# AhauBioinformatics/IDDGCN

Measured on AMD Instinct MI355X. Metric: adjacency edges/s per IDDGCN training step (pos fwd + neg fwd + bwd + Adam), higher is better.
Workload: dtype f32

## Files before the change

### iddgcn_amd/csrc/iddgcn_hip.hip

```cpp
#include <hip/hip_runtime.h>
#include <stdint.h>

#include <type_traits>

#include "../../include/iddgcn.h"

typedef float f32x4 __attribute__((ext_vector_type(4)));
typedef float f32x16 __attribute__((ext_vector_type(16)));
typedef _Float16 f16x4 __attribute__((ext_vector_type(4)));
typedef _Float16 f16x8 __attribute__((ext_vector_type(8)));
typedef __bf16 bf16x8 __attribute__((ext_vector_type(8)));
typedef __bf16 bf16x4 __attribute__((ext_vector_type(4)));
typedef short s16x4 __attribute__((ext_vector_type(4)));
typedef unsigned int u32x2 __attribute__((ext_vector_type(2)));
typedef unsigned int u32x4 __attribute__((ext_vector_type(4)));

#define MAX_R 8
#define EPS_BCE 1e-7f

namespace {

__device__ __forceinline__ float sigmoidf_(float x) { return 1.0f / (1.0f + expf(-x)); }
__device__ __forceinline__ float sigmoid_fast(float x) { return __builtin_amdgcn_rcpf(1.0f + __expf(-x)); }

// ... 2191 lines not shown
            tr_read_asm(fa[k][1], pa + 512 * k + 4 * PT);
            tr_read_asm(fb[k][0], pb0 + 512 * k);
            tr_read_asm(fb[k][1], pb0 + 512 * k + 4 * PT);
        }
        tie6(fa);
        tie6(fb);
        const bf16x8 a0 = frag(fa[0]), a1 = frag(fa[1]), a2 = frag(fa[2]);
#pragma unroll
        for (int cj = 0; cj < 8; ++cj) {
            if (cj + 1 < 8) {
                const char* pb = pb0 + 64 * (cj + 1);
#pragma unroll
                for (int k = 0; k < 3; ++k) {
                    tr_read_asm(fn[k][0], pb + 512 * k);
                    tr_read_asm(fn[k][1], pb + 512 * k + 4 * PT);
                }
            }
            const bf16x8 b0 = frag(fb[0]), b1 = frag(fb[1]), b2 = frag(fb[2]);
            f32x16 c;
#pragma unroll
            for (int j = 0; j < 16; ++j) c[j] = 0.f;
            c = __builtin_amdgcn_mfma_f32_32x32x16_bf16(a0, b2, c, 0, 0, 0);
            c = __builtin_amdgcn_mfma_f32_32x32x16_bf16(a2, b0, c, 0, 0, 0);
            c = __builtin_amdgcn_mfma_f32_32x32x16_bf16(a1, b1, c, 0, 0, 0);
            c = __builtin_amdgcn_mfma_f32_32x32x16_bf16(a0, b1, c, 0, 0, 0);
            c = __builtin_amdgcn_mfma_f32_32x32x16_bf16(a1, b0, c, 0, 0, 0);
            acc[cj] = __builtin_amdgcn_mfma_f32_32x32x16_bf16(a0, b0, acc[cj] + c, 0, 0, 0);
            __builtin_amdgcn_sched_barrier(0);
            if (cj + 1 < 8) {
                tie6(fn);
#pragma unroll
                for (int k = 0; k < 3; ++k) {
                    fb[k][0] = fn[k][0];
                    fb[k][1] = fn[k][1];
                }
            }
        }
    };

    if (nt > 0) {
        stage(0, 0);
        const int n1 = nt > 1 ? stage(1, 1) : 0;
        wait_newest(n1);
        convert(0);
        asm volatile("s_waitcnt lgkmcnt(0)" ::: "memory");
        __syncthreads();
    }
#define TB3_LOOP(LATE)                                                               \
    {                                                                                \
        int b = 0;                                                                   \
        for (long long t = 0; t < nt; ++t) {                                         \
            const int b1 = b == 2 ? 0 : b + 1, b2 = b1 == 2 ? 0 : b1 + 1;            \
            const int n2 = t + 2 < nt ? stage(t + 2, b2) : 0;                        \
            if (LATE && t + 1 < nt) {                                                \
                wait_newest(n2);                                                     \
                convert(b1);                                                         \
            }                                                                        \
            mfma_tile(b);                                                            \
            if (!LATE && t + 1 < nt) {                                               \
                wait_newest(n2);                                                     \
                convert(b1);                                                         \
            }                                                                        \
            asm volatile("s_waitcnt lgkmcnt(0)" ::: "memory");                       \
            __builtin_amdgcn_s_barrier();                                            \
            asm volatile("" ::: "memory");                                           \
            b = b1;                                                                  \
        }                                                                            \
    }
    if (late) TB3_LOOP(true) else TB3_LOOP(false)
#undef TB3_LOOP
    float* out = slab + (long long)blockIdx.x * D * D;
    const int i = lane & 31, h = lane >> 5;
#pragma unroll
    for (int cj = 0; cj < 8; ++cj)
#pragma unroll
        for (int j = 0; j < 16; ++j) {
            const int row = 32 * wave + (j & 3) + 8 * (j >> 2) + 4 * h;
            out[row * D + 32 * cj + i] = acc[cj][j];
        }
}

namespace st3 {
constexpr int D = 256, TR = 32, DP = 1536, XP = 768, DOB = TR * DP, XB = TR * XP, BUF = DOB + XB, NBUF = 2;
}
template <int PS>
__device__ __forceinline__ void tr_read3(v4s16 (&d)[3], unsigned a) {
    asm volatile("ds_read_b64_tr_b16 %0, %3\n\tds_read_b64_tr_b16 %1, %3 offset:%4\n\tds_read_b64_tr_b16 %2, %3 offset:%5"
                 : "=&v"(d[0]), "=&v"(d[1]), "=&v"(d[2])
                 : "v"(a), "i"(PS), "i"(2 * PS)
                 : "memory");
}
__device__ __forceinline__ bf16x8 cat_tr(const v4s16& a, const v4s16& b) {
    return __builtin_bit_cast(bf16x8, __builtin_shufflevector(a, b, 0, 1, 2, 3, 4, 5, 6, 7));
}
__device__ __forceinline__ float bf_at(const u32x2& v, int q) {
    const unsigned w = v[q >> 1];
    return __builtin_bit_cast(float, (q & 1) ? (w & 0xffff0000u) : (w << 16));
}
__global__ __launch_bounds__(512) void sigma_tn_b3_kernel(long long M, int tiles_per_block, int n_ranges,
                                                          const float* __restrict__ dO, float* __restrict__ X,
                                                          const float* __restrict__ S, float* __restrict__ slab) {
    using namespace st3;
    static_assert(NBUF * BUF <= 160 * 1024, "LDS budget");
    __shared__ __attribute__((aligned(16))) char lds[NBUF * BUF];
    const int lane = threadIdx.x & 63;
    const int wave = __builtin_amdgcn_readfirstlane(threadIdx.x >> 6);
    const int bx = blockIdx.x;
    const int half = (bx >> 3) & 1;
    const int range = ((bx >> 4) << 3) | (bx & 7);
    if (range >= n_ranges) return;
    const long long ntiles = (M + TR - 1) / TR;
    const long long t_beg = (long long)range * tiles_per_block;
    long long t_end = t_beg + tiles_per_block;
    if (t_end > ntiles) t_end = ntiles;
    const int i16 = lane & 15, g = lane >> 4;
    const int c0 = 128 * half + 16 * wave;
    const unsigned lds0 = lds_u32(lds);
    auto fresh_lane = [&]() __attribute__((always_inline)) {
        int l = lane;
        asm volatile("" : "+v"(l));
        return l;
    };

    bf16x8 w0[8], w1[8], w2[8];
#pragma unroll
    for (int q = 0; q < 8; ++q)
#pragma unroll
        for (int e = 0; e < 8; ++e) {
            __bf16 a, b, c;
            split3(S[(c0 + i16) * D + 32 * q + 8 * g + e], a, b, c);
            w0[q][e] = a;
            w1[q][e] = b;
            w2[q][e] = c;
        }
    f32x4 tacc[2][8];
#pragma unroll
    for (int mb = 0; mb < 2; ++mb)
#pragma unroll
        for (int nb = 0; nb < 8; ++nb) tacc[mb][nb] = f32x4{0.f, 0.f, 0.f, 0.f};

    auto stage = [&](long long t, int bb, int wave) __attribute__((always_inline)) -> int {
        const int lane = fresh_lane();
        char* base = lds + bb * BUF;
        const long long t0 = t * TR;
        if (t0 + TR <= M) {
#pragma unroll
            for (int j = 0; j < 4; ++j) {
                const int r = 4 * wave + j;
                __builtin_amdgcn_global_load_lds((gbl_vptr)(dO + (t0 + r) * D + lane * 4), (lds_vptr)(base + r * DP), 16,
                                                 0, 0);
            }
#pragma unroll
            for (int p = 0; p < 2; ++p) {
                const int r = 4 * wave + 2 * p;
                __builtin_amdgcn_global_load_lds(
                    (gbl_vptr)(X + (t0 + r + (lane >> 5)) * D + 128 * half + (lane & 31) * 4),
                    (lds_vptr)(base + DOB + r * XP), 16, 0, 0);
            }
            return 6;
        }
        int n = 0;
#pragma unroll
        for (int j = 0; j < 4; ++j) {
            const int r = 4 * wave + j;
            const long long e = t0 + r;
            char* xr = base + DOB + (r & ~1) * XP + 512 * (r & 1);
            if (e < M) {
                __builtin_amdgcn_global_load_lds((gbl_vptr)(dO + e * D + lane * 4), (lds_vptr)(base + r * DP), 16, 0, 0);
                if (lane < 32)
                    __builtin_amdgcn_global_load_lds((gbl_vptr)(X + e * D + 128 * half + lane * 4), (lds_vptr)xr, 16, 0,
                                                     0);
                n += 2;
            } else {
                st4(reinterpret_cast<float*>(base + r * DP) + lane * 4, f32x4{0.f, 0.f, 0.f, 0.f});
                if (lane < 32) st4(reinterpret_cast<float*>(xr) + lane * 4, f32x4{0.f, 0.f, 0.f, 0.f});
            }
        }
        return n;
    };
    auto convert = [&](int bb, int wave) __attribute__((always_inline)) {
        char* base = lds + bb * BUF;
        const int lane = fresh_lane();
        u32x4 v[6];
#pragma unroll
        for (int j = 0; j < 4; ++j)
            asm volatile("ds_read_b128 %0, %1" : "=v"(v[j]) : "v"(lds_u32(base + (4 * wave + j) * DP) + 16 * lane) : "memory");
#pragma unroll
        for (int p = 0; p < 2; ++p)
            asm volatile("ds_read_b128 %0, %1"
                         : "=v"(v[4 + p])
                         : "v"(lds_u32(base + DOB + (4 * wave + 2 * p) * XP) + 16 * lane)
                         : "memory");
        asm volatile("s_waitcnt lgkmcnt(0)" : "+v"(v[0]), "+v"(v[1]), "+v"(v[2]), "+v"(v[3]), "+v"(v[4]), "+v"(v[5])::"memory");
#pragma unroll
        for (int j = 0; j < 4; ++j) {
            const int r = 4 * wave + j;
            char* row = base + r * DP + 16 * ((lane >> 1) ^ stn_sw(r)) + 8 * (lane & 1);
            bf16x4 p0, p1, p2;
            split3x4(__builtin_bit_cast(f32x4, v[j]), p0, p1, p2);
            *reinterpret_cast<bf16x4*>(row) = p0;
            *reinterpret_cast<bf16x4*>(row + 512) = p1;
            *reinterpret_cast<bf16x4*>(row + 1024) = p2;
        }
#pragma unroll
        for (int p = 0; p < 2; ++p) {
            const int r = 4 * wave + 2 * p + (lane >> 5);
            char* row = base + DOB + r * XP + 16 * (((lane & 31) >> 1) ^ stn_sw(r)) + 8 * (lane & 1);
            bf16x4 p0, p1, p2;
            split3x4(__builtin_bit_cast(f32x4, v[4 + p]), p0, p1, p2);
            *reinterpret_cast<bf16x4*>(row) = p0;
            *reinterpret_cast<bf16x4*>(row + 256) = p1;
            *reinterpret_cast<bf16x4*>(row + 512) = p2;
        }
    };
    auto mfma_sigma = [&](int bb, f32x4 (&acc)[2]) __attribute__((always_inline)) {
        const int lane = fresh_lane();
        const int i16 = lane & 15, g = lane >> 4, swi = stn_sw(i16), sa = swi >> 2, sl = swi & 3;
        const unsigned rb0 = lds0 + bb * BUF + i16 * DP + 16 * (g ^ sl);
        const unsigned ad0 = rb0 + 64 * (0 ^ sa), ad1 = rb0 + 64 * (1 ^ sa), ad2 = rb0 + 64 * (2 ^ sa),
                       ad3 = rb0 + 64 * (3 ^ sa);
        f32x4 hi0 = {0.f, 0.f, 0.f, 0.f}, lo0 = hi0, hi1 = hi0, lo1 = hi0;
        u32x4 fx[2][3], fy[2][3];
        asm volatile("s_waitcnt lgkmcnt(0)" ::: "memory");
#define ST3_LOADQ(Q, S_, AD)                                                                              \
        asm volatile("ds_read_b128 %0, %6 offset:%7\n\tds_read_b128 %1, %6 offset:%8\n\t"                 \
                     "ds_read_b128 %2, %6 offset:%9\n\tds_read_b128 %3, %6 offset:%10\n\t"                \
                     "ds_read_b128 %4, %6 offset:%11\n\tds_read_b128 %5, %6 offset:%12"                   \
                     : "=&v"(fx[S_][0]), "=&v"(fx[S_][1]), "=&v"(fx[S_][2]), "=&v"(fy[S_][0]), "=&v"(fy[S_][1]),  \
                       "=&v"(fy[S_][2])                                                                  \
                     : "v"(AD), "i"(256 * ((Q) >> 2)), "i"(256 * ((Q) >> 2) + 512),                       \
                       "i"(256 * ((Q) >> 2) + 1024), "i"(256 * ((Q) >> 2) + 16 * DP),                     \
                       "i"(256 * ((Q) >> 2) + 16 * DP + 512), "i"(256 * ((Q) >> 2) + 16 * DP + 1024)      \
                     : "memory")
        ST3_LOADQ(0, 0, ad0);
#pragma unroll
        for (int q = 0; q < 8; ++q) {
            const int S_ = q & 1;
            if (q + 1 < 8) {
                switch (q) {
                    case 0: ST3_LOADQ(1, 1, ad1); break;
                    case 1: ST3_LOADQ(2, 0, ad2); break;
                    case 2: ST3_LOADQ(3, 1, ad3); break;
                    case 3: ST3_LOADQ(4, 0, ad0); break;
                    case 4: ST3_LOADQ(5, 1, ad1); break;
                    case 5: ST3_LOADQ(6, 0, ad2); break;
                    default: ST3_LOADQ(7, 1, ad3); break;
                }
                asm volatile("s_waitcnt lgkmcnt(6)"
                             : "+v"(fx[S_][0]), "+v"(fx[S_][1]), "+v"(fx[S_][2]), "+v"(fy[S_][0]), "+v"(fy[S_][1]),
                               "+v"(fy[S_][2])::"memory");
            } else {
                asm volatile("s_waitcnt lgkmcnt(0)"
                             : "+v"(fx[S_][0]), "+v"(fx[S_][1]), "+v"(fx[S_][2]), "+v"(fy[S_][0]), "+v"(fy[S_][1]),
                               "+v"(fy[S_][2])::"memory");
            }
            const bf16x8 x0 = __builtin_bit_cast(bf16x8, fx[S_][0]), x1 = __builtin_bit_cast(bf16x8, fx[S_][1]),
                         x2 = __builtin_bit_cast(bf16x8, fx[S_][2]);
            const bf16x8 y0 = __builtin_bit_cast(bf16x8, fy[S_][0]), y1 = __builtin_bit_cast(bf16x8, fy[S_][1]),
                         y2 = __builtin_bit_cast(bf16x8, fy[S_][2]);
            lo0 = __builtin_amdgcn_mfma_f32_16x16x32_bf16(w0[q], x2, lo0, 0, 0, 0);
            lo1 = __builtin_amdgcn_mfma_f32_16x16x32_bf16(w0[q], y2, lo1, 0, 0, 0);
            lo0 = __builtin_amdgcn_mfma_f32_16x16x32_bf16(w2[q], x0, lo0, 0, 0, 0);
            lo1 = __builtin_amdgcn_mfma_f32_16x16x32_bf16(w2[q], y0, lo1, 0, 0, 0);
            lo0 = __builtin_amdgcn_mfma_f32_16x16x32_bf16(w1[q], x1, lo0, 0, 0, 0);
            lo1 = __builtin_amdgcn_mfma_f32_16x16x32_bf16(w1[q], y1, lo1, 0, 0, 0);
            lo0 = __builtin_amdgcn_mfma_f32_16x16x32_bf16(w0[q], x1, lo0, 0, 0, 0);
            lo1 = __builtin_amdgcn_mfma_f32_16x16x32_bf16(w0[q], y1, lo1, 0, 0, 0);
            lo0 = __builtin_amdgcn_mfma_f32_16x16x32_bf16(w1[q], x0, lo0, 0, 0, 0);
            lo1 = __builtin_amdgcn_mfma_f32_16x16x32_bf16(w1[q], y0, lo1, 0, 0, 0);
            hi0 = __builtin_amdgcn_mfma_f32_16x16x32_bf16(w0[q], x0, hi0, 0, 0, 0);
            hi1 = __builtin_amdgcn_mfma_f32_16x16x32_bf16(w0[q], y0, hi1, 0, 0, 0);
        }
#undef ST3_LOADQ
        acc[0] = hi0 + lo0;
        acc[1] = hi1 + lo1;
    };
    auto mfma_tn = [&](int bb) __attribute__((always_inline)) {
        const int lane = fresh_lane();
        const int tra = 8 * (lane >> 4) + ((lane >> 2) & 3), trq = tra + 4;
        const int swa = stn_sw(tra), swq = stn_sw(trq);
        const int tb = (lane & 3) >> 1;
        const unsigned xoa = tra * XP + 16 * (tb ^ (swa & 1)) + 8 * (lane & 1),
                       xoq = trq * XP + 16 * (tb ^ (swq & 1)) + 8 * (lane & 1);
        const unsigned doa = tra * DP + 16 * (tb ^ (swa & 1)) + 8 * (lane & 1) + 256 * (wave >> 2),
                       doq = trq * DP + 16 * (tb ^ (swq & 1)) + 8 * (lane & 1) + 256 * (wave >> 2);
        const int swa_e = swa & 14, swq_e = swq & 14;
        const unsigned db = lds0 + bb * BUF, xb = db + DOB;
        v4s16 xa[2][2][3], fb[2][2][3];
#pragma unroll
        for (int mb = 0; mb < 2; ++mb) {
            const int cx = 4 * (wave & 3) + 2 * mb;
            tr_read3<256>(xa[mb][0], xb + xoa + 16 * (cx ^ swa_e));
            tr_read3<256>(xa[mb][1], xb + xoq + 16 * (cx ^ swq_e));
        }
        tr_read3<512>(fb[0][0], db + doa + 16 * (0 ^ swa_e));
        tr_read3<512>(fb[0][1], db + doq + 16 * (0 ^ swq_e));
        asm volatile("s_waitcnt lgkmcnt(0)"
                     : "+v"(xa[0][0][0]), "+v"(xa[0][0][1]), "+v"(xa[0][0][2]), "+v"(xa[0][1][0]), "+v"(xa[0][1][1]),
                       "+v"(xa[0][1][2]), "+v"(xa[1][0][0]), "+v"(xa[1][0][1]), "+v"(xa[1][0][2]), "+v"(xa[1][1][0]),
                       "+v"(xa[1][1][1]), "+v"(xa[1][1][2]), "+v"(fb[0][0][0]), "+v"(fb[0][0][1]), "+v"(fb[0][0][2]),
                       "+v"(fb[0][1][0]), "+v"(fb[0][1][1]), "+v"(fb[0][1][2])::"memory");
        bf16x8 a[2][3];
#pragma unroll
        for (int mb = 0; mb < 2; ++mb)
#pragma unroll
            for (int j = 0; j < 3; ++j) a[mb][j] = cat_tr(xa[mb][0][j], xa[mb][1][j]);
#pragma unroll
        for (int nb = 0; nb < 8; ++nb) {
            const int s = nb & 1;
            if (nb + 1 < 8) {
                tr_read3<512>(fb[s ^ 1][0], db + doa + 16 * ((2 * (nb + 1)) ^ swa_e));
                tr_read3<512>(fb[s ^ 1][1], db + doq + 16 * ((2 * (nb + 1)) ^ swq_e));
            }
            const bf16x8 b0 = cat_tr(fb[s][0][0], fb[s][1][0]), b1 = cat_tr(fb[s][0][1], fb[s][1][1]),
                         b2 = cat_tr(fb[s][0][2], fb[s][1][2]);
            const f32x4 z = {0.f, 0.f, 0.f, 0.f};
            f32x4 e0 = __builtin_amdgcn_mfma_f32_16x16x32_bf16(a[0][0], b2, z, 0, 0, 0);
            f32x4 e1 = __builtin_amdgcn_mfma_f32_16x16x32_bf16(a[1][0], b2, z, 0, 0, 0);
            e0 = __builtin_amdgcn_mfma_f32_16x16x32_bf16(a[0][2], b0, e0, 0, 0, 0);
            e1 = __builtin_amdgcn_mfma_f32_16x16x32_bf16(a[1][2], b0, e1, 0, 0, 0);
            e0 = __builtin_amdgcn_mfma_f32_16x16x32_bf16(a[0][1], b1, e0, 0, 0, 0);
            e1 = __builtin_amdgcn_mfma_f32_16x16x32_bf16(a[1][1], b1, e1, 0, 0, 0);
            e0 = __builtin_amdgcn_mfma_f32_16x16x32_bf16(a[0][0], b1, e0, 0, 0, 0);
            e1 = __builtin_amdgcn_mfma_f32_16x16x32_bf16(a[1][0], b1, e1, 0, 0, 0);
            e0 = __builtin_amdgcn_mfma_f32_16x16x32_bf16(a[0][1], b0, e0, 0, 0, 0);
            e1 = __builtin_amdgcn_mfma_f32_16x16x32_bf16(a[1][1], b0, e1, 0, 0, 0);
            tacc[0][nb] = __builtin_amdgcn_mfma_f32_16x16x32_bf16(a[0][0], b0, tacc[0][nb] + e0, 0, 0, 0);
            tacc[1][nb] = __builtin_amdgcn_mfma_f32_16x16x32_bf16(a[1][0], b0, tacc[1][nb] + e1, 0, 0, 0);
            __builtin_amdgcn_sched_barrier(0);
            if (nb + 1 < 8)
                asm volatile("s_waitcnt lgkmcnt(0)"
                             : "+v"(fb[s ^ 1][0][0]), "+v"(fb[s ^ 1][0][1]), "+v"(fb[s ^ 1][0][2]), "+v"(fb[s ^ 1][1][0]),
                               "+v"(fb[s ^ 1][1][1]), "+v"(fb[s ^ 1][1][2])::"memory");
        }
    };
    auto epilogue = [&](long long t, int bb, const f32x4 (&acc)[2]) __attribute__((always_inline)) -> int {
        const int lane = fresh_lane();
        const int i16 = lane & 15, g = lane >> 4, swi = stn_sw(i16);
        const unsigned xb = lds0 + bb * BUF + DOB + 16 * ((2 * wave + (g >> 1)) ^ swi) + 8 * (g & 1);
        u32x2 xr[2][3];
#pragma unroll
        for (int rb = 0; rb < 2; ++rb)
            asm volatile("ds_read_b64 %0, %3\n\tds_read_b64 %1, %3 offset:256\n\tds_read_b64 %2, %3 offset:512"
                         : "=&v"(xr[rb][0]), "=&v"(xr[rb][1]), "=&v"(xr[rb][2])
                         : "v"(xb + (16 * rb + i16) * XP)
                         : "memory");
        asm volatile("s_waitcnt lgkmcnt(0)"
                     : "+v"(xr[0][0]), "+v"(xr[0][1]), "+v"(xr[0][2]), "+v"(xr[1][0]), "+v"(xr[1][1]), "+v"(xr[1][2])::"memory");
        const long long row0 = t * TR;
        const long long left = M - row0;
        const unsigned nbytes = (unsigned)((left < TR ? left : TR) * D * 4);
        const __amdgpu_buffer_rsrc_t rc =
            __builtin_amdgcn_make_buffer_rsrc(reinterpret_cast<char*>(X) + row0 * D * 4, (short)0, nbytes, 0x00020000);
#pragma unroll
        for (int rb = 0; rb < 2; ++rb) {
            const int r = 16 * rb + i16;
            f32x4 v = acc[rb];
#pragma unroll
            for (int q = 0; q < 4; ++q) {
                const float x = (bf_at(xr[rb][0], q) + bf_at(xr[rb][1], q)) + bf_at(xr[rb][2], q);
                v[q] = v[q] * (x * (1.0f - x));
            }
            __builtin_amdgcn_raw_buffer_store_b128(v, rc, (r * D + 128 * half + 16 * wave + 4 * g) * 4, 0, 0);
        }
        return 2;
    };

    if (t_beg < t_end) {
        stage(t_beg, 0, wave);
        asm volatile("s_waitcnt vmcnt(0)" ::: "memory");
        convert(0, wave);
        asm volatile("s_waitcnt lgkmcnt(0)" ::: "memory");
        __syncthreads();
        {
            int b = 0;
            const bool stager = wave < 4;
            for (long long t = t_beg; t < t_end; ++t) {
                const bool more = t + 1 < t_end;
                if (more && stager) {
                    stage(t + 1, b ^ 1, wave);
                    stage(t + 1, b ^ 1, wave + 4);
                }
                f32x4 acc[2];
                mfma_sigma(b, acc);
                const int ns = epilogue(t, b, acc);
                mfma_tn(b);
                if (more && stager) {
                    wait_vm(ns);
                    convert(b ^ 1, wave);
                    convert(b ^ 1, wave + 4);
                }
                asm volatile("s_waitcnt lgkmcnt(0)" ::: "memory");
                __builtin_amdgcn_s_barrier();
                asm volatile("" ::: "memory");
                b ^= 1;
            }
        }
    }
    float* out = slab + (long long)range * D * D;
#pragma unroll
    for (int mb = 0; mb < 2; ++mb)
#pragma unroll
        for (int nb = 0; nb < 8; ++nb)
#pragma unroll
            for (int j = 0; j < 4; ++j) {
                const int row = 128 * half + 32 * (wave & 3) + 16 * mb + 4 * g + j;
                out[row * D + 128 * (wave >> 2) + 16 * nb + i16] = tacc[mb][nb][j];
            }
}

template <int D>
__global__ __launch_bounds__(D) void gemm_tn_narrow_kernel(long long M, long long rows_per_block, int R,
                                                           const float* __restrict__ A,
                                                           const float* __restrict__ dz,
                                                           float* __restrict__ slab) {
    const int d = threadIdx.x;
    float acc[MAX_R], accb[MAX_R];
#pragma unroll
    for (int r = 0; r < MAX_R; ++r) acc[r] = accb[r] = 0.f;
    const long long r_beg = (long long)blockIdx.x * rows_per_block;
    long long r_end = r_beg + rows_per_block;
    if (r_end > M) r_end = M;
    for (long long e = r_beg; e < r_end; ++e) {
        const float a = A[e * D + d];
#pragma unroll
        for (int r = 0; r < MAX_R; ++r)
            if (r < R) {
                const float z = dz[e * R + r];
                acc[r] += a * z;
                accb[r] += z;
            }
    }
    float* out = slab + (long long)blockIdx.x * (D + 1) * R;
#pragma unroll
    for (int r = 0; r < MAX_R; ++r)
        if (r < R) {
            out[d * R + r] = acc[r];
            if (d == 0) out[D * R + r] = accb[r];
        }
}

template <int D>
__global__ __launch_bounds__(256) void alpha_kernel(int M, int R, const float* __restrict__ X,
                                                    const int* __restrict__ x_idx, const float* __restrict__ Wa,
                                                    const float* __restrict__ ba, float* __restrict__ S_out,
                                                    float* __restrict__ W_out) {
    constexpr int LPR = D / 4;
    constexpr int K = LPR < MAX_R ? LPR : MAX_R;
    const int sub = threadIdx.x % LPR;
    float wa[4][MAX_R];
#pragma unroll
    for (int j = 0; j < 4; ++j)
#pragma unroll
        for (int r = 0; r < MAX_R; ++r) wa[j][r] = r < R ? Wa[(sub * 4 + j) * R + r] : 0.f;
    float bav[MAX_R];
#pragma unroll
    for (int r = 0; r < MAX_R; ++r) bav[r] = r < R ? ba[r] : 0.f;
    const long long gstride = (long long)gridDim.x * (blockDim.x / LPR);
    for (long long row = ((long long)blockIdx.x * blockDim.x + threadIdx.x) / LPR; row < M; row += gstride) {
        const long long src = x_idx ? (long long)x_idx[row] : row;
        const f32x4 x = ld4(X + src * D + sub * 4);
        float z[MAX_R];
#pragma unroll
        for (int r0 = 0; r0 < MAX_R; r0 += K) {
            float part[K];
#pragma unroll
            for (int q = 0; q < K; ++q) {
                const int r = r0 + q;
                part[q] = 0.f;
#pragma unroll
                for (int j = 0; j < 4; ++j) part[q] = fmaf(x[j], wa[j][r], part[q]);
            }
            const float tot = multi_reduce<LPR, K>(part, sub);
#pragma unroll
            for (int q = 0; q < K; ++q) z[r0 + q] = __shfl(tot, (threadIdx.x & ~(LPR - 1) & 63) + q * (LPR / K), 64);
        }
        if (sub != 0) continue;
        float mx = -INFINITY;
#pragma unroll
        for (int r = 0; r < MAX_R; ++r)
            if (r < R) {
                z[r] += bav[r];
                mx = fmaxf(mx, z[r]);
            }
        float sum = 0.f;
#pragma unroll
        for (int r = 0; r < MAX_R; ++r)
            if (r < R) {
                z[r] = expf(z[r] - mx);
                sum += z[r];
// ... 2150 lines not shown
    if (a->planes) return IDDGCN_E_BAD_ARG;
    RowGemmP p = to_p(*a);
    p.accumulate = 0;
    auto al16 = [](const void* q) { return ((uintptr_t)q & 15) == 0; };
    if (a->R == 8 && a->v_idx && !a->coef_idx && !a->a_idx && !a->b_trans && !dsig && al16(a->A) && al16(a->C) &&
        al16(a->coef) && al16(a->V) && (a->v_rel_stride & 3) == 0) {
        launch_fwd_gather8((hipStream_t)stream, p);
        return launch_status();
    }
    V3Sel sel;
    sel.nv = a->R == 0 ? 0 : a->R == 1 ? 1 : a->R == 2 ? 2 : a->R <= 4 ? 4 : 8;
    sel.aux = dsig;
    sel.hc = a->R > 0;
    RowGemmBatch pb;
    pb.p[0] = p;
    launch_v3((hipStream_t)stream, pb, 1, sel, true);
    return launch_status();
}

int iddgcn_gemm_tn_bf16(void* stream, long long M, int d, const void* A, const void* B, float* slab, int n_blocks,
                        float* C, int accumulate) {
    if (d != 256) return IDDGCN_E_BAD_DIM;
    if (M < 0 || n_blocks < 1 || !A || !B || !slab || !C) return IDDGCN_E_BAD_ARG;
    hipStream_t st = (hipStream_t)stream;
    long long rpb = (M + n_blocks - 1) / n_blocks;
    rpb = ((rpb + 31) / 32) * 32;
    if (rpb < 32) rpb = 32;
    hipLaunchKernelGGL(gemm_tn256_bf16t_kernel, dim3(n_blocks), dim3(512), 0, st, M, rpb,
                       (const __bf16*)A, (const __bf16*)B, slab);
    int rc = launch_status();
    if (rc) return rc;
    const long long n = (long long)d * d;
    launch_reduce_slabs(st, n_blocks, n, slab, C, accumulate, 1.0f);
    return launch_status();
}

int iddgcn_sigma_tn_ranges(long long M) {
    const long long nt = (M + stn::TR - 1) / stn::TR;
    long long nr = nt < 128 ? nt : 128;
    if (nr < 1) nr = 1;
    const long long tpb = (nt + nr - 1) / nr > 0 ? (nt + nr - 1) / nr : 1;
    nr = (nt + tpb - 1) / tpb;
    return (int)((nr + 7) / 8 * 8 > 0 ? (nr + 7) / 8 * 8 : 8);
}

int iddgcn_sigma_tn_bf16(void* stream, long long M, int d, const void* dO, void* X, const float* S, float* slab,
                         long long slab_floats, float* dS, int precision) {
    if (d != 256) return IDDGCN_E_BAD_DIM;
    if (precision != IDDGCN_GEMM_EXACT_F32 && precision != IDDGCN_GEMM_SPLIT_F16 && precision != IDDGCN_GEMM_BF16X3 &&
        precision != IDDGCN_GEMM_BF16)
        return IDDGCN_E_BAD_ARG;
    if (M < 0 || !S || !slab || !dS || (M > 0 && (!dO || !X))) return IDDGCN_E_BAD_ARG;
    if (((uintptr_t)dO & 15) || ((uintptr_t)X & 15)) return IDDGCN_E_BAD_ARG;
    hipStream_t st = (hipStream_t)stream;
    const long long nt = (M + stn::TR - 1) / stn::TR;
    const int nr = iddgcn_sigma_tn_ranges(M);
    const long long tpb = nt > 0 ? (nt + nr - 1) / nr : 1;
    const long long n = (long long)d * d;
    if (slab_floats < nr * n) return IDDGCN_E_BAD_ARG;
    if (precision == IDDGCN_GEMM_BF16)
        hipLaunchKernelGGL(sigma_tn_bf16_kernel<true>, dim3((unsigned)(2 * nr)), dim3(512), 0, st, M, (int)tpb, nr,
                           (const __bf16*)dO, (__bf16*)X, S, slab);
    else
        hipLaunchKernelGGL(sigma_tn_bf16_kernel<false>, dim3((unsigned)(2 * nr)), dim3(512), 0, st, M, (int)tpb, nr,
                           (const __bf16*)dO, (__bf16*)X, S, slab);
    int rc = launch_status();
    if (rc) return rc;
    launch_reduce_slabs(st, nr, n, slab, dS, 0, 1.0f);
    return launch_status();
}

int iddgcn_sigma_tn_f32(void* stream, long long M, int d, const float* dO, float* X, const float* S, float* slab,
                        long long slab_floats, float* dS, int precision) {
    if (d != 256) return IDDGCN_E_BAD_DIM;
    if (precision != IDDGCN_GEMM_BF16X3) return IDDGCN_E_BAD_ARG;
    if (M < 0 || !S || !slab || !dS || (M > 0 && (!dO || !X))) return IDDGCN_E_BAD_ARG;
    if (((uintptr_t)dO & 15) || ((uintptr_t)X & 15)) return IDDGCN_E_BAD_ARG;
    hipStream_t st = (hipStream_t)stream;
    const long long nt = (M + st3::TR - 1) / st3::TR;
    const int nr = iddgcn_sigma_tn_ranges(M);
    const long long tpb = nt > 0 ? (nt + nr - 1) / nr : 1;
    const long long n = (long long)d * d;
    if (slab_floats < nr * n) return IDDGCN_E_BAD_ARG;
    hipLaunchKernelGGL(sigma_tn_b3_kernel, dim3((unsigned)(2 * nr)), dim3(512), 0, st, M, (int)tpb, nr, dO, X, S, slab);
    int rc = launch_status();
    if (rc) return rc;
    launch_reduce_slabs(st, nr, n, slab, dS, 0, 1.0f);
    return launch_status();
}

int iddgcn_combine_bf16(void* stream, int M, int d, int R, const float* Y, const int* idx, const float* coef,
                        const float* V, long long v_rel_stride, void* out) {
    return run_combine_out<true, false>(stream, M, d, R, Y, idx, coef, V, v_rel_stride, out);
}

int iddgcn_combine_planes_f32(void* stream, int M, int d, int R, const float* Y, const int* idx, const float* coef,
                              const float* V, long long v_rel_stride, void* out) {
    return run_combine_out<false, true>(stream, M, d, R, Y, idx, coef, V, v_rel_stride, out);
}

int iddgcn_distmult_bce_bf16(void* stream, long long T, int d, int R, const float* Xh, const int* h_idx,
                             const void* Xt, const int* t_idx, const int* r_idx, const float* rel, const float* y,
                             float scale, float* p_out, float* s_out, float* ds_out, void* do_out,
                             float* drel_slab, float* loss_slab, int n_blocks) {
    if (d != 256) return IDDGCN_E_BAD_DIM;
    if (R < 1 || R > MAX_R) return IDDGCN_E_BAD_REL;
    if (T < 0 || n_blocks < 1 || !Xh || !h_idx || !Xt || !r_idx || !rel) return IDDGCN_E_BAD_ARG;
    if (y && (!ds_out || !do_out || !drel_slab || !loss_slab)) return IDDGCN_E_BAD_ARG;
    if (T == 0) return 0;
    hipLaunchKernelGGL((distmult_kernel<256, true>), dim3(n_blocks), dim3(256), 0, (hipStream_t)stream, T, R, Xh, h_idx,
                       (const float*)Xt, t_idx, r_idx, rel, y, scale, p_out, s_out, ds_out, (float*)do_out, drel_slab,
                       loss_slab);
    return launch_status();
}

int iddgcn_distmult_bce_heads_bf16(void* stream, int n_nodes, int d, int R, const int* seg_ptr, const int* perm,
                                   const float* Xh, const void* Xt, const int* r_idx, const float* rel,
                                   const float* y, float scale, float* p_out, float* s_out, float* ds_out,
                                   void* do_out, float* dXh, float* drel_slab, float* loss_slab, int n_blocks) {
    if (d != 256) return IDDGCN_E_BAD_DIM;
    if (R < 1 || R > MAX_R) return IDDGCN_E_BAD_REL;
    if (n_nodes < 0 || n_blocks < 1 || !seg_ptr || !perm || !Xh || !Xt || !r_idx || !rel || !do_out || !dXh ||
        !drel_slab || !loss_slab)
        return IDDGCN_E_BAD_ARG;
    hipStream_t st = (hipStream_t)stream;
#define HKB(RT) hipLaunchKernelGGL((distmult_heads_kernel<256, RT, true>), dim3(n_blocks), dim3(256), 0, st, n_nodes, R, seg_ptr, perm, Xh, (const float*)Xt, r_idx, rel, y, scale, p_out, s_out, ds_out, (float*)do_out, dXh, drel_slab, loss_slab)
    if (R <= 1) HKB(1);
    else if (R <= 2) HKB(2);
    else if (R <= 4) HKB(4);
    else HKB(8);
#undef HKB
    return launch_status();
}

int iddgcn_tail_seg_reduce_head_bf16(void* stream, int n_nodes, int d, int R, const int* seg_ptr, const float* W,
                                     const void* dO, const float* P, long long p_rel_stride, float* dP,
                                     long long dp_rel_stride, float* dsum, float* dWedge, const float* head_dO,
                                     const float* Wn, float* dwh) {
    if (d != 256) return IDDGCN_E_BAD_DIM;
    if (R != 8) return IDDGCN_E_BAD_REL;
    if (n_nodes < 0 || !seg_ptr || !W || !dO || !P || !dP || !dWedge || !head_dO || !Wn || !dwh)
        return IDDGCN_E_BAD_ARG;
    if (n_nodes == 0) return 0;
    launch_tail_mfma8((hipStream_t)stream, n_nodes, seg_ptr, W, dO, P, p_rel_stride, dP, dp_rel_stride, dsum, dWedge,
                      head_dO, Wn, dwh);
    return launch_status();
}

int iddgcn_head_dz_f32(void* stream, int n_nodes, int R, const float* Ssm, const float* W, const int* hseg_ptr,
                       const int* hperm, const float* dWedge, const float* dwh, float* dz) {
    if (R < 1 || R > MAX_R) return IDDGCN_E_BAD_REL;
    if (n_nodes < 0 || !Ssm || !W || !hseg_ptr || !hperm || !dWedge || !dwh || !dz) return IDDGCN_E_BAD_ARG;
    if (n_nodes == 0) return 0;
    hipLaunchKernelGGL(head_dz_kernel, dim3((unsigned)(((long long)n_nodes * 8 + 255) / 256)), dim3(256), 0,
                       (hipStream_t)stream, n_nodes, R, Ssm, W, hseg_ptr, hperm, dWedge, dwh, dz);
    return launch_status();
}

int iddgcn_tail_seg_reduce_bf16(void* stream, int n_nodes, int d, int R, const int* seg_ptr, const int* h_idx,
                                const float* W, const void* dO, const float* P, long long p_rel_stride, float* dP,
                                long long dp_rel_stride, float* dsum, float* dWedge) {
    if (d != 256) return IDDGCN_E_BAD_DIM;
    if (R < 1 || R > MAX_R) return IDDGCN_E_BAD_REL;
    if (n_nodes < 0 || !seg_ptr || !W || !dO || !P || !dP || !dWedge) return IDDGCN_E_BAD_ARG;
    if (n_nodes == 0) return 0;
    hipStream_t st = (hipStream_t)stream;
    const unsigned grid = grid_for(n_nodes, 64);
// ... 29 lines not shown
```

Before: 81.46 million.

## Add dedicated TN waves to sigma_tn kernel and rebalance column work

Raises the fused sigma/TN backward kernel from 8 to 12 waves per block. The 4 new waves only compute the X^T·dO product for 12 of the 16 column blocks, while the original 8 waves keep the sigma MFMA, epilogue and staging and handle the remaining 4 column blocks. The goal is to take most of the TN accumulation off the critical path of the sigma waves so the two matrix products overlap. The sigma LDS reads are also reorganised into a finer-grained interleaved prefetch between MFMA groups. The cost is higher register pressure from the 768-thread launch bound and a larger block, which may reduce occupancy.

```diff
diff --git a/iddgcn_amd/csrc/iddgcn_hip.hip b/iddgcn_amd/csrc/iddgcn_hip.hip
--- a/iddgcn_amd/csrc/iddgcn_hip.hip
+++ b/iddgcn_amd/csrc/iddgcn_hip.hip
@@ -2297,6 +2297,11 @@
 
 namespace st3 {
 constexpr int D = 256, TR = 32, DP = 1536, XP = 768, DOB = TR * DP, XB = TR * XP, BUF = DOB + XB, NBUF = 2;
+constexpr int NBT = 12;
+template <int N>
+struct ic {
+    static constexpr int v = N;
+};
 }
 template <int PS>
 __device__ __forceinline__ void tr_read3(v4s16 (&d)[3], unsigned a) {
@@ -2312,7 +2317,7 @@
     const unsigned w = v[q >> 1];
     return __builtin_bit_cast(float, (q & 1) ? (w & 0xffff0000u) : (w << 16));
 }
-__global__ __launch_bounds__(512) void sigma_tn_b3_kernel(long long M, int tiles_per_block, int n_ranges,
+__global__ __launch_bounds__(768) void sigma_tn_b3_kernel(long long M, int tiles_per_block, int n_ranges,
                                                           const float* __restrict__ dO, float* __restrict__ X,
                                                           const float* __restrict__ S, float* __restrict__ slab) {
     using namespace st3;
@@ -2328,7 +2333,7 @@
     const long long t_beg = (long long)range * tiles_per_block;
     long long t_end = t_beg + tiles_per_block;
     if (t_end > ntiles) t_end = ntiles;
-    const int i16 = lane & 15, g = lane >> 4;
+    const int n_t = __builtin_amdgcn_readfirstlane(t_end > t_beg ? (int)(t_end - t_beg) : 0);
     const int c0 = 128 * half + 16 * wave;
     const unsigned lds0 = lds_u32(lds);
     auto fresh_lane = [&]() __attribute__((always_inline)) {
@@ -2337,22 +2342,8 @@
         return l;
     };
 
+    const bool tn_wave = wave >= 8;
     bf16x8 w0[8], w1[8], w2[8];
-#pragma unroll
-    for (int q = 0; q < 8; ++q)
-#pragma unroll
-        for (int e = 0; e < 8; ++e) {
-            __bf16 a, b, c;
-            split3(S[(c0 + i16) * D + 32 * q + 8 * g + e], a, b, c);
-            w0[q][e] = a;
-            w1[q][e] = b;
-            w2[q][e] = c;
-        }
-    f32x4 tacc[2][8];
-#pragma unroll
-    for (int mb = 0; mb < 2; ++mb)
-#pragma unroll
-        for (int nb = 0; nb < 8; ++nb) tacc[mb][nb] = f32x4{0.f, 0.f, 0.f, 0.f};
 
     auto stage = [&](long long t, int bb, int wave) __attribute__((always_inline)) -> int {
         const int lane = fresh_lane();
@@ -2431,85 +2422,78 @@
     auto mfma_sigma = [&](int bb, f32x4 (&acc)[2]) __attribute__((always_inline)) {
         const int lane = fresh_lane();
         const int i16 = lane & 15, g = lane >> 4, swi = stn_sw(i16), sa = swi >> 2, sl = swi & 3;
-        const unsigned rb0 = lds0 + bb * BUF + i16 * DP + 16 * (g ^ sl);
-        const unsigned ad0 = rb0 + 64 * (0 ^ sa), ad1 = rb0 + 64 * (1 ^ sa), ad2 = rb0 + 64 * (2 ^ sa),
-                       ad3 = rb0 + 64 * (3 ^ sa);
+        const unsigned sb = lds0 + bb * BUF, rb0 = i16 * DP + 16 * (g ^ sl) + 64 * sa;
+        auto adq = [&](int q) __attribute__((always_inline)) {
+            unsigned r = rb0;
+            asm volatile("" : "+v"(r));
+            return sb + 256 * (q >> 2) + (r ^ (64 * (q & 3)));
+        };
         f32x4 hi0 = {0.f, 0.f, 0.f, 0.f}, lo0 = hi0, hi1 = hi0, lo1 = hi0;
-        u32x4 fx[2][3], fy[2][3];
+        u32x4 x0, y0, x1, y1, x2, y2;
         asm volatile("s_waitcnt lgkmcnt(0)" ::: "memory");
-#define ST3_LOADQ(Q, S_, AD)                                                                              \
-        asm volatile("ds_read_b128 %0, %6 offset:%7\n\tds_read_b128 %1, %6 offset:%8\n\t"                 \
-                     "ds_read_b128 %2, %6 offset:%9\n\tds_read_b128 %3, %6 offset:%10\n\t"                \
-                     "ds_read_b128 %4, %6 offset:%11\n\tds_read_b128 %5, %6 offset:%12"                   \
-                     : "=&v"(fx[S_][0]), "=&v"(fx[S_][1]), "=&v"(fx[S_][2]), "=&v"(fy[S_][0]), "=&v"(fy[S_][1]),  \
-                       "=&v"(fy[S_][2])                                                                  \
-                     : "v"(AD), "i"(256 * ((Q) >> 2)), "i"(256 * ((Q) >> 2) + 512),                       \
-                       "i"(256 * ((Q) >> 2) + 1024), "i"(256 * ((Q) >> 2) + 16 * DP),                     \
-                       "i"(256 * ((Q) >> 2) + 16 * DP + 512), "i"(256 * ((Q) >> 2) + 16 * DP + 1024)      \
-                     : "memory")
-        ST3_LOADQ(0, 0, ad0);
+#define ST3_LD2(DX, DY, AD, OFF)                                                                               \
+        do {                                                                                                   \
+            asm volatile("ds_read_b128 %0, %1 offset:%2" : "=v"(DX) : "v"(AD), "i"(OFF) : "memory");           \
+            asm volatile("ds_read_b128 %0, %1 offset:%2" : "=v"(DY) : "v"(AD), "i"((OFF) + 16 * DP) : "memory"); \
+        } while (0)
+        {
+            const unsigned ad = adq(0);
+            ST3_LD2(x0, y0, ad, 0);
+            ST3_LD2(x2, y2, ad, 1024);
+            ST3_LD2(x1, y1, ad, 512);
+        }
 #pragma unroll
         for (int q = 0; q < 8; ++q) {
-            const int S_ = q & 1;
-            if (q + 1 < 8) {
-                switch (q) {
-                    case 0: ST3_LOADQ(1, 1, ad1); break;
-                    case 1: ST3_LOADQ(2, 0, ad2); break;
-                    case 2: ST3_LOADQ(3, 1, ad3); break;
-                    case 3: ST3_LOADQ(4, 0, ad0); break;
-                    case 4: ST3_LOADQ(5, 1, ad1); break;
-                    case 5: ST3_LOADQ(6, 0, ad2); break;
-                    default: ST3_LOADQ(7, 1, ad3); break;
-                }
-                asm volatile("s_waitcnt lgkmcnt(6)"
-                             : "+v"(fx[S_][0]), "+v"(fx[S_][1]), "+v"(fx[S_][2]), "+v"(fy[S_][0]), "+v"(fy[S_][1]),
-                               "+v"(fy[S_][2])::"memory");
-            } else {
-                asm volatile("s_waitcnt lgkmcnt(0)"
-                             : "+v"(fx[S_][0]), "+v"(fx[S_][1]), "+v"(fx[S_][2]), "+v"(fy[S_][0]), "+v"(fy[S_][1]),
-                               "+v"(fy[S_][2])::"memory");
-            }
-            const bf16x8 x0 = __builtin_bit_cast(bf16x8, fx[S_][0]), x1 = __builtin_bit_cast(bf16x8, fx[S_][1]),
-                         x2 = __builtin_bit_cast(bf16x8, fx[S_][2]);
-            const bf16x8 y0 = __builtin_bit_cast(bf16x8, fy[S_][0]), y1 = __builtin_bit_cast(bf16x8, fy[S_][1]),
-                         y2 = __builtin_bit_cast(bf16x8, fy[S_][2]);
-            lo0 = __builtin_amdgcn_mfma_f32_16x16x32_bf16(w0[q], x2, lo0, 0, 0, 0);
-            lo1 = __builtin_amdgcn_mfma_f32_16x16x32_bf16(w0[q], y2, lo1, 0, 0, 0);
-            lo0 = __builtin_amdgcn_mfma_f32_16x16x32_bf16(w2[q], x0, lo0, 0, 0, 0);
-            lo1 = __builtin_amdgcn_mfma_f32_16x16x32_bf16(w2[q], y0, lo1, 0, 0, 0);
-            lo0 = __builtin_amdgcn_mfma_f32_16x16x32_bf16(w1[q], x1, lo0, 0, 0, 0);
-            lo1 = __builtin_amdgcn_mfma_f32_16x16x32_bf16(w1[q], y1, lo1, 0, 0, 0);
-            lo0 = __builtin_amdgcn_mfma_f32_16x16x32_bf16(w0[q], x1, lo0, 0, 0, 0);
-            lo1 = __builtin_amdgcn_mfma_f32_16x16x32_bf16(w0[q], y1, lo1, 0, 0, 0);
-            lo0 = __builtin_amdgcn_mfma_f32_16x16x32_bf16(w1[q], x0, lo0, 0, 0, 0);
-            lo1 = __builtin_amdgcn_mfma_f32_16x16x32_bf16(w1[q], y0, lo1, 0, 0, 0);
-            hi0 = __builtin_amdgcn_mfma_f32_16x16x32_bf16(w0[q], x0, hi0, 0, 0, 0);
-            hi1 = __builtin_amdgcn_mfma_f32_16x16x32_bf16(w0[q], y0, hi1, 0, 0, 0);
-        }
-#undef ST3_LOADQ
+            const bool more = q + 1 < 8;
+            const unsigned nad = adq(more ? q + 1 : q);
+            asm volatile("s_waitcnt lgkmcnt(0)" : "+v"(x0), "+v"(y0), "+v"(x2), "+v"(y2), "+v"(x1), "+v"(y1)::"memory");
+            const bf16x8 fx0 = __builtin_bit_cast(bf16x8, x0), fy0 = __builtin_bit_cast(bf16x8, y0);
+            const bf16x8 fx1 = __builtin_bit_cast(bf16x8, x1), fy1 = __builtin_bit_cast(bf16x8, y1);
+            lo0 = __builtin_amdgcn_mfma_f32_16x16x32_bf16(w0[q], __builtin_bit_cast(bf16x8, x2), lo0, 0, 0, 0);
+            lo1 = __builtin_amdgcn_mfma_f32_16x16x32_bf16(w0[q], __builtin_bit_cast(bf16x8, y2), lo1, 0, 0, 0);
+            __builtin_amdgcn_sched_barrier(0);
+            if (more) ST3_LD2(x2, y2, nad, 1024);
+            lo0 = __builtin_amdgcn_mfma_f32_16x16x32_bf16(w2[q], fx0, lo0, 0, 0, 0);
+            lo1 = __builtin_amdgcn_mfma_f32_16x16x32_bf16(w2[q], fy0, lo1, 0, 0, 0);
+            lo0 = __builtin_amdgcn_mfma_f32_16x16x32_bf16(w1[q], fx1, lo0, 0, 0, 0);
+            lo1 = __builtin_amdgcn_mfma_f32_16x16x32_bf16(w1[q], fy1, lo1, 0, 0, 0);
+            lo0 = __builtin_amdgcn_mfma_f32_16x16x32_bf16(w0[q], fx1, lo0, 0, 0, 0);
+            lo1 = __builtin_amdgcn_mfma_f32_16x16x32_bf16(w0[q], fy1, lo1, 0, 0, 0);
+            __builtin_amdgcn_sched_barrier(0);
+            if (more) ST3_LD2(x1, y1, nad, 512);
+            lo0 = __builtin_amdgcn_mfma_f32_16x16x32_bf16(w1[q], fx0, lo0, 0, 0, 0);
+            lo1 = __builtin_amdgcn_mfma_f32_16x16x32_bf16(w1[q], fy0, lo1, 0, 0, 0);
+            hi0 = __builtin_amdgcn_mfma_f32_16x16x32_bf16(w0[q], fx0, hi0, 0, 0, 0);
+            hi1 = __builtin_amdgcn_mfma_f32_16x16x32_bf16(w0[q], fy0, hi1, 0, 0, 0);
+            __builtin_amdgcn_sched_barrier(0);
+            if (more) ST3_LD2(x0, y0, nad, 0);
+        }
+#undef ST3_LD2
         acc[0] = hi0 + lo0;
         acc[1] = hi1 + lo1;
     };
-    auto mfma_tn = [&](int bb) __attribute__((always_inline)) {
+    auto mfma_tn = [&](int bb, int xg, int nb0, auto nbc, auto dbc, auto& tacc) __attribute__((always_inline)) {
+        constexpr int NB = decltype(nbc)::v;
+        constexpr bool DB = decltype(dbc)::v != 0;
         const int lane = fresh_lane();
         const int tra = 8 * (lane >> 4) + ((lane >> 2) & 3), trq = tra + 4;
         const int swa = stn_sw(tra), swq = stn_sw(trq);
         const int tb = (lane & 3) >> 1;
         const unsigned xoa = tra * XP + 16 * (tb ^ (swa & 1)) + 8 * (lane & 1),
                        xoq = trq * XP + 16 * (tb ^ (swq & 1)) + 8 * (lane & 1);
-        const unsigned doa = tra * DP + 16 * (tb ^ (swa & 1)) + 8 * (lane & 1) + 256 * (wave >> 2),
-                       doq = trq * DP + 16 * (tb ^ (swq & 1)) + 8 * (lane & 1) + 256 * (wave >> 2);
+        const unsigned doa = tra * DP + 16 * (tb ^ (swa & 1)) + 8 * (lane & 1),
+                       doq = trq * DP + 16 * (tb ^ (swq & 1)) + 8 * (lane & 1);
         const int swa_e = swa & 14, swq_e = swq & 14;
         const unsigned db = lds0 + bb * BUF, xb = db + DOB;
         v4s16 xa[2][2][3], fb[2][2][3];
 #pragma unroll
         for (int mb = 0; mb < 2; ++mb) {
-            const int cx = 4 * (wave & 3) + 2 * mb;
+            const int cx = 4 * xg + 2 * mb;
             tr_read3<256>(xa[mb][0], xb + xoa + 16 * (cx ^ swa_e));
             tr_read3<256>(xa[mb][1], xb + xoq + 16 * (cx ^ swq_e));
         }
-        tr_read3<512>(fb[0][0], db + doa + 16 * (0 ^ swa_e));
-        tr_read3<512>(fb[0][1], db + doq + 16 * (0 ^ swq_e));
+        tr_read3<512>(fb[0][0], db + doa + 16 * ((2 * nb0) ^ swa_e));
+        tr_read3<512>(fb[0][1], db + doq + 16 * ((2 * nb0) ^ swq_e));
         asm volatile("s_waitcnt lgkmcnt(0)"
                      : "+v"(xa[0][0][0]), "+v"(xa[0][0][1]), "+v"(xa[0][0][2]), "+v"(xa[0][1][0]), "+v"(xa[0][1][1]),
                        "+v"(xa[0][1][2]), "+v"(xa[1][0][0]), "+v"(xa[1][0][1]), "+v"(xa[1][0][2]), "+v"(xa[1][1][0]),
@@ -2521,11 +2505,12 @@
 #pragma unroll
             for (int j = 0; j < 3; ++j) a[mb][j] = cat_tr(xa[mb][0][j], xa[mb][1][j]);
 #pragma unroll
-        for (int nb = 0; nb < 8; ++nb) {
-            const int s = nb & 1;
-            if (nb + 1 < 8) {
-                tr_read3<512>(fb[s ^ 1][0], db + doa + 16 * ((2 * (nb + 1)) ^ swa_e));
-                tr_read3<512>(fb[s ^ 1][1], db + doq + 16 * ((2 * (nb + 1)) ^ swq_e));
+        for (int i = 0; i < NB; ++i) {
+            const int s = DB ? (i & 1) : 0, sn = DB ? (s ^ 1) : 0;
+            const bool more = i + 1 < NB;
+            if (DB && more) {
+                tr_read3<512>(fb[sn][0], db + doa + 16 * ((2 * (nb0 + i + 1)) ^ swa_e));
+                tr_read3<512>(fb[sn][1], db + doq + 16 * ((2 * (nb0 + i + 1)) ^ swq_e));
             }
             const bf16x8 b0 = cat_tr(fb[s][0][0], fb[s][1][0]), b1 = cat_tr(fb[s][0][1], fb[s][1][1]),
                          b2 = cat_tr(fb[s][0][2], fb[s][1][2]);
@@ -2540,13 +2525,17 @@
             e1 = __builtin_amdgcn_mfma_f32_16x16x32_bf16(a[1][0], b1, e1, 0, 0, 0);
             e0 = __builtin_amdgcn_mfma_f32_16x16x32_bf16(a[0][1], b0, e0, 0, 0, 0);
             e1 = __builtin_amdgcn_mfma_f32_16x16x32_bf16(a[1][1], b0, e1, 0, 0, 0);
-            tacc[0][nb] = __builtin_amdgcn_mfma_f32_16x16x32_bf16(a[0][0], b0, tacc[0][nb] + e0, 0, 0, 0);
-            tacc[1][nb] = __builtin_amdgcn_mfma_f32_16x16x32_bf16(a[1][0], b0, tacc[1][nb] + e1, 0, 0, 0);
+            tacc[0][i] = __builtin_amdgcn_mfma_f32_16x16x32_bf16(a[0][0], b0, tacc[0][i] + e0, 0, 0, 0);
+            tacc[1][i] = __builtin_amdgcn_mfma_f32_16x16x32_bf16(a[1][0], b0, tacc[1][i] + e1, 0, 0, 0);
             __builtin_amdgcn_sched_barrier(0);
-            if (nb + 1 < 8)
+            if (!DB && more) {
+                tr_read3<512>(fb[0][0], db + doa + 16 * ((2 * (nb0 + i + 1)) ^ swa_e));
+                tr_read3<512>(fb[0][1], db + doq + 16 * ((2 * (nb0 + i + 1)) ^ swq_e));
+            }
+            if (more)
                 asm volatile("s_waitcnt lgkmcnt(0)"
-                             : "+v"(fb[s ^ 1][0][0]), "+v"(fb[s ^ 1][0][1]), "+v"(fb[s ^ 1][0][2]), "+v"(fb[s ^ 1][1][0]),
-                               "+v"(fb[s ^ 1][1][1]), "+v"(fb[s ^ 1][1][2])::"memory");
+                             : "+v"(fb[sn][0][0]), "+v"(fb[sn][0][1]), "+v"(fb[sn][0][2]), "+v"(fb[sn][1][0]),
+                               "+v"(fb[sn][1][1]), "+v"(fb[sn][1][2])::"memory");
         }
     };
     auto epilogue = [&](long long t, int bb, const f32x4 (&acc)[2]) __attribute__((always_inline)) -> int {
@@ -2581,17 +2570,68 @@
         return 2;
     };
 
-    if (t_beg < t_end) {
+    if (tn_wave) {
+        f32x4 tacc[2][NBT];
+#pragma unroll
+        for (int mb = 0; mb < 2; ++mb)
+#pragma unroll
+            for (int nb = 0; nb < NBT; ++nb) tacc[mb][nb] = f32x4{0.f, 0.f, 0.f, 0.f};
+        if (n_t > 0) {
+            __builtin_amdgcn_s_barrier();
+            asm volatile("" ::: "memory");
+        }
+        int b = 0;
+        for (int it = 0; it < n_t; ++it) {
+            mfma_tn(b, wave - 8, 0, ic<NBT>{}, ic<1>{}, tacc);
+            __builtin_amdgcn_s_barrier();
+            asm volatile("" ::: "memory");
+            b ^= 1;
+        }
+        float* out = slab + (long long)range * D * D;
+        const int i16 = fresh_lane() & 15, g = fresh_lane() >> 4;
+#pragma unroll
+        for (int mb = 0; mb < 2; ++mb)
+#pragma unroll
+            for (int nb = 0; nb < NBT; ++nb)
+#pragma unroll
+                for (int j = 0; j < 4; ++j) {
+                    const int row = 128 * half + 32 * (wave - 8) + 16 * mb + 4 * g + j;
+                    out[row * D + 16 * nb + i16] = tacc[mb][nb][j];
+                }
+        return;
+    }
+    {
+        const int i16 = lane & 15, g = lane >> 4;
+#pragma unroll
+        for (int q = 0; q < 8; ++q)
+#pragma unroll
+            for (int e = 0; e < 8; ++e) {
+                __bf16 a, b, c;
+                split3(S[(c0 + i16) * D + 32 * q + 8 * g + e], a, b, c);
+                w0[q][e] = a;
+                w1[q][e] = b;
+                w2[q][e] = c;
+            }
+    }
+    const int own_nb0 = NBT + 2 * (wave >> 2);
+    f32x4 tacc[2][2];
+#pragma unroll
+    for (int mb = 0; mb < 2; ++mb)
+#pragma unroll
+        for (int i = 0; i < 2; ++i) tacc[mb][i] = f32x4{0.f, 0.f, 0.f, 0.f};
+    if (n_t > 0) {
         stage(t_beg, 0, wave);
         asm volatile("s_waitcnt vmcnt(0)" ::: "memory");
         convert(0, wave);
         asm volatile("s_waitcnt lgkmcnt(0)" ::: "memory");
-        __syncthreads();
+        __builtin_amdgcn_s_barrier();
+        asm volatile("" ::: "memory");
         {
             int b = 0;
             const bool stager = wave < 4;
-            for (long long t = t_beg; t < t_end; ++t) {
-                const bool more = t + 1 < t_end;
+            for (int it = 0; it < n_t; ++it) {
+                const long long t = t_beg + it;
+                const bool more = it + 1 < n_t;
                 if (more && stager) {
                     stage(t + 1, b ^ 1, wave);
                     stage(t + 1, b ^ 1, wave + 4);
@@ -2599,7 +2639,7 @@
                 f32x4 acc[2];
                 mfma_sigma(b, acc);
                 const int ns = epilogue(t, b, acc);
-                mfma_tn(b);
+                mfma_tn(b, wave & 3, own_nb0, ic<2>{}, ic<0>{}, tacc);
                 if (more && stager) {
                     wait_vm(ns);
                     convert(b ^ 1, wave);
@@ -2613,14 +2653,15 @@
         }
     }
     float* out = slab + (long long)range * D * D;
+    const int i16 = fresh_lane() & 15, g = fresh_lane() >> 4;
 #pragma unroll
     for (int mb = 0; mb < 2; ++mb)
 #pragma unroll
-        for (int nb = 0; nb < 8; ++nb)
+        for (int i = 0; i < 2; ++i)
 #pragma unroll
             for (int j = 0; j < 4; ++j) {
                 const int row = 128 * half + 32 * (wave & 3) + 16 * mb + 4 * g + j;
-                out[row * D + 128 * (wave >> 2) + 16 * nb + i16] = tacc[mb][nb][j];
+                out[row * D + 16 * (own_nb0 + i) + i16] = tacc[mb][i][j];
             }
 }
 
@@ -4937,7 +4978,7 @@
     const long long tpb = nt > 0 ? (nt + nr - 1) / nr : 1;
     const long long n = (long long)d * d;
     if (slab_floats < nr * n) return IDDGCN_E_BAD_ARG;
-    hipLaunchKernelGGL(sigma_tn_b3_kernel, dim3((unsigned)(2 * nr)), dim3(512), 0, st, M, (int)tpb, nr, dO, X, S, slab);
+    hipLaunchKernelGGL(sigma_tn_b3_kernel, dim3((unsigned)(2 * nr)), dim3(768), 0, st, M, (int)tpb, nr, dO, X, S, slab);
     int rc = launch_status();
     if (rc) return rc;
     launch_reduce_slabs(st, nr, n, slab, dS, 0, 1.0f);
```

Result: faster. 83.16 million, median of 6 (+2.1%).
